# atoms-ufrj/atomsmm

Measured on AMD Instinct MI355X. Metric: ns/day on 100k-atom TIP3P RESPA box; near-nonbonded HBM GB/s vs 8 TB/s peak, higher is better.
Workload: dtype f64

## Files before the change

### atomsmm_amd/csrc/abi.hip

```cpp
#include <algorithm>
#include <cmath>
#include <cstring>
#include <numeric>

#include "amm_ctx.h"
#include "cluster.h"

int amm_pair_setup_grid(amm_ctx *ctx, PairForce *pf);
static bool amm_family_allows_cluster(int family, int flags) {
    const bool tab_family = family == AMM_NEAR_NONE || family == AMM_NEAR_SHIFT || family == AMM_NEAR_FSWITCH || family == AMM_DAMPED || family == AMM_NONBONDED;
    return tab_family && !(flags & (AMM_GROUP_LJ | AMM_GROUP_Q));
}
int amm_bonded_arity(int kind);
int amm_bonded_npar(int kind);

static thread_local std::string g_error;
void amm_set_error(const std::string &msg) { g_error = msg; }

static PairForce *get_pair(amm_ctx *ctx, int id) {
    if (!ctx || id < 0 || id >= (int)ctx->forces.size() || ctx->forces[id].type != 1) {
        amm_set_error("invalid pair force id");
        return nullptr;
    }
    return ctx->forces[id].pair;
// ... 1758 lines not shown
        amm_set_error("amm_set_option: null argument");
        return 1;
    }
    const std::string k(name);
    const int v = (int)value;
    if (k == "cluster") ctx->opt_cluster = v;
    else if (k == "hybrid") ctx->opt_hybrid = v;
    else if (k == "small_group") ctx->opt_small_group = v;
    else if (k == "mixed_terms") ctx->opt_mixed_terms = v;
    else if (k == "rest_skin_factor") ctx->opt_rest_skin_factor = value;
    else if (k == "tab") ctx->opt_tab = v;
    else if (k == "site_trips") ctx->site_trips = v != 0;
    else if (k == "lanes_per_row") ctx->opt_lpa = v;
    else if (k == "build_parts") ctx->opt_parts = v;
    else if (k == "build_split") ctx->opt_build_split = v;
    else if (k == "unroll") ctx->opt_unroll = v;
    else if (k == "dual_unroll") ctx->opt_dual_unroll = v;
    else if (k == "tab_block") ctx->opt_tab_bs = v;
    else if (k == "tab_dual_block") ctx->opt_tab_dual_bs = v;
    else if (k == "no_dual") ctx->opt_no_dual = v;
    else if (k == "fuse_rows") ctx->opt_fuse_rows = v;
    else if (k == "row_phases") ctx->opt_row_phases = v;
    else if (k == "group_candidates") ctx->opt_group_candidates = v;
    else if (k == "positions_private") ctx->opt_positions_private = v;
    else if (k == "site_tab") ctx->opt_site_tab = v;
    else if (k == "no_defer") ctx->opt_no_defer = v;
    else if (k == "terms_from") ctx->opt_terms_from = v;
    else if (k == "no_term_lanes") ctx->opt_no_term_lanes = v;
    else if (k == "fuse_epilogue") ctx->opt_fuse_epilogue = v;
    else if (k == "comm_timeout") ctx->opt_comm_timeout = value;
// ... 63 lines not shown
```

### atomsmm_amd/csrc/amm_ctx.h

```cpp
#pragma once
#include <hip/hip_runtime.h>

#include <cstdint>
#include <string>
#include <vector>

#include "../../include/atomsmm_hip.h"

#define AMM_WAVE 64
#define AMM_MAX_PRE 6
#define AMM_DERIV_LAMBDA 1024
#define AMM_MAX_GROUPS 33

void amm_set_error(const std::string &msg);
#define AMM_HIP(call)                                                                            \
    do {                                                                                         \
        hipError_t e_ = (call);                                                                  \
        if (e_ != hipSuccess) {                                                                  \
            amm_set_error(std::string(#call) + ": " + hipGetErrorString(e_));                    \
            return 1;                                                                            \
        }                                                                                        \
    } while (0)

struct PairTab {
// ... 253 lines not shown
    int opt_chargeless = 1;
    int opt_fuse_epilogue = 1;
    const EpiPlan *epi_request = nullptr;
    bool epi_done = false;
    long long n_epilogues = 0;
    long long n_state_exchanges = 0;
    std::vector<const double *> own_only;
    long long n_copies_current = 0;
    int opt_cluster = 1;
    int opt_hybrid = 1;
    double opt_rest_skin_factor = 2.0;
    int opt_mixed_terms = 1;
    int opt_small_group = 1;
    bool creating_rest = false;
    int opt_tab = 1;
    int opt_build_split = 0;
    int opt_lpa = 0, opt_parts = 0, opt_unroll = 2, opt_dual_unroll = 2, opt_tab_bs = 0, opt_tab_dual_bs = 0;
    int opt_site_tab = 1;
    CZeroRows zero_rows = CZeroRows{0, nullptr, nullptr, nullptr};
    int opt_positions_private = 0;
    int opt_group_candidates = 1;
    int opt_row_phases = 1;
    int opt_fuse_rows = 1;
    int opt_no_dual = 0, opt_no_defer = 0, opt_terms_from = 8192, opt_no_term_lanes = 0;
    ListWatch watched[AMM_MAX_WATCH];
    int n_watched = 0;
    int device = 0;
    hipStream_t stream = nullptr;
    Box box;
    int rank = 0, world = 1;
// ... 111 lines not shown
```

### atomsmm_amd/csrc/cluster.h

```cpp
#pragma once
#include "amm_ctx.h"

struct ClusterList {
    int nc = 0;
    const int *d_first = nullptr;
    const int *d_rest = nullptr;
    int nrest = 0;
    bool built = false;
    CellGrid grid;
    int capc = 0;
    int parts = 1;
    int *d_slice_cells = nullptr;
    int split_parts = 0;
    double rext = 0;
    double rlist_build = 0, rnear_build = 0, skin = 0;
    int *d_cell_count = nullptr, *d_cell_start = nullptr, *d_cell_members = nullptr;
    int *d_cperm = nullptr;
    int *d_aperm = nullptr;
    float4 *d_pos4f = nullptr;
    double *d_xref = nullptr;
    int c_begin = 0, c_end = 0;
    int cap = 0;
    int lpa = 8;
    int *d_nl = nullptr, *d_nnb = nullptr, *d_nnb_near = nullptr;
    int *d_flags = nullptr;
    unsigned long long *d_counters = nullptr;
    unsigned long long *d_blockstats = nullptr;
    int *d_ticket = nullptr;
    long checked_epoch = -1, pre_epoch = -1;
    const double *checked_pos = nullptr, *pre_pos = nullptr;
    PairForce *sorted_for = nullptr;
// ... 19 lines not shown
```

### atomsmm_amd/csrc/cluster.hip

```cpp
#include <algorithm>
#include <cmath>
#include <cstdio>
#include <cstdlib>
#include <cstring>
#include <type_traits>
#include <vector>

#include "amm_ctx.h"
#include "bonded_terms.h"
#include "cluster.h"
#include "device_utils.h"
#include "pair_math.h"
#include "pair_tab.h"

#ifndef AMM_EXP_NOLJ
#define AMM_EXP_NOLJ 0
#endif

__device__ double amm_erfcx_table_dev_c[AMM_ERFCX_NI * AMM_ERFCX_NC];
static bool g_erfcx_uploaded_c[64] = {false};

void amm_cluster_classify(int n, const std::vector<int> &ptr, const std::vector<int> &idx, std::vector<int> &mol_first, std::vector<int> &rest) {
    mol_first.clear();
    rest.clear();
// ... 77 lines not shown
#pragma unroll
    for (int k = 0; k < 3; ++k) sh[k] = cwrap1(pos[3 * i0 + k], box.L[k], box.invL[k]) - pos[3 * i0 + k];
#pragma unroll
    for (int a = 0; a < 3; ++a) {
        const int i = i0 + a;
        double4 p;
        p.x = csorted_image(pos[3 * i], pos[3 * i0], sh[0], box.L[0], box.invL[0]);
        p.y = csorted_image(pos[3 * i + 1], pos[3 * i0 + 1], sh[1], box.L[1], box.invL[1]);
        p.z = csorted_image(pos[3 * i + 2], pos[3 * i0 + 2], sh[2], box.L[2], box.invL[2]);
        p.w = q[i];
        posq_s[3 * c + a] = p;
        lj_s[3 * c + a] = make_double2(hsig[i], seps2[i]);
    }
}

__global__ void __launch_bounds__(256) k_csort_gather(int ncell, int nc, const int *__restrict__ start, const int *__restrict__ members,
                                                      int capc, int *cperm, int *aperm, const double *__restrict__ pos, Box box,
                                                      float4 *pos4f, const int *flags, int *wflags, int force, const double *__restrict__ q,
                                                      const double *__restrict__ hsig, const double *__restrict__ seps2, double4 *posq_s,
                                                      double2 *lj_s, float rext, const double *__restrict__ site_eps,
                                                      const int *__restrict__ first, CZeroRows Z, int copies_current, double *xref,
                                                      int c_begin, int c_end, int *slice_cells) {
    const int gid = blockIdx.x * blockDim.x + threadIdx.x;
    if (gid < Z.n) {
        const int i = Z.idx[gid];
        if (Z.f0) Z.f0[3 * i] = Z.f0[3 * i + 1] = Z.f0[3 * i + 2] = 0.0;
        if (Z.f1) Z.f1[3 * i] = Z.f1[3 * i + 1] = Z.f1[3 * i + 2] = 0.0;
    }
    if (!force && !flags[0]) {
        if (!copies_current && posq_s && gid < nc) cgather_one(gid, cfirst(first, cperm[gid]), pos, box, q, hsig, seps2, posq_s, lj_s);
        return;
    }
    const int wave = gid >> 6, lane = threadIdx.x & 63;
    if (wave >= ncell) return;
    const int b = start[wave];
    const int cnt = min(start[wave + 1] - b, capc);
    if (lane == 0 && c_begin < c_end) {
        if (b <= c_begin && c_begin < start[wave + 1]) slice_cells[0] = wave;
        if (b <= c_end - 1 && c_end - 1 < start[wave + 1]) slice_cells[1] = wave;
    }
    const int *mem = members + (size_t)wave * capc;
    for (int a0 = 0; a0 < cnt; a0 += 64) {
        const int a = a0 + lane;
        const int me = a < cnt ? mem[a] : 0x7fffffff;
        int rank = 0;
        for (int k0 = 0; k0 < cnt; k0 += 64) {
            const int kk = k0 + lane;
            const int other = kk < cnt ? mem[kk] : 0x7fffffff;
            const int nk = min(64, cnt - k0);
            for (int jj = 0; jj < nk; ++jj) rank += __builtin_amdgcn_readlane(other, jj) < me;
        }
        if (a >= cnt) continue;
        const int sl = b + rank;
        cperm[sl] = me;
        const int i0 = cfirst(first, me);
        double sh[3], p0[3];
#pragma unroll
        for (int k = 0; k < 3; ++k) {
            p0[k] = pos[3 * i0 + k];
            sh[k] = cwrap1(p0[k], box.L[k], box.invL[k]) - p0[k];
        }
        float ext2 = 0.f;
        int sites = 0;
        float4 pf[3];
#pragma unroll
        for (int t = 0; t < 3; ++t) {
            const int i = i0 + t;
            aperm[3 * sl + t] = i;
            const double x = csorted_image(pos[3 * i], p0[0], sh[0], box.L[0], box.invL[0]);
            const double y = csorted_image(pos[3 * i + 1], p0[1], sh[1], box.L[1], box.invL[1]);
// ... 7 lines not shown
            const float dx = pf[t].x - pf[0].x, dy = pf[t].y - pf[0].y, dz = pf[t].z - pf[0].z;
            ext2 = fmaxf(ext2, dx * dx + dy * dy + dz * dz);
            if (site_eps[i] != 0.0) sites |= 1 << t;
            if (posq_s) {
                posq_s[3 * sl + t] = make_double4(x, y, z, q[i]);
                lj_s[3 * sl + t] = make_double2(hsig[i], seps2[i]);
            }
        }
        const float ext = sqrtf(ext2) * 1.000001f + 1e-6f;
        if (!(ext <= rext)) wflags[7] = 1;
        pf[0].w = ext;
        pf[1].w = __int_as_float(sites);
        pos4f[3 * sl] = pf[0];
        pos4f[3 * sl + 1] = pf[1];
        pos4f[3 * sl + 2] = pf[2];
    }
}

struct CBoxF {
    float L[3], invL[3];
};

#ifndef CB_BATCH
#define CB_BATCH 5
#endif
#define CB_COARSE 256
#define CB_QCAP 256
__device__ __forceinline__ int cq_wrap(int i) { return i & (CB_QCAP - 1); }
typedef float v2f __attribute__((ext_vector_type(2)));

__device__ void cfinish_build_block(int *flags, unsigned long long *counters, const unsigned long long *blockstats, int nblocks, int count_only) {
    __shared__ unsigned long long sh_part[4][3];
    unsigned long long sum = 0, mx = 0, nr = 0;
    for (int b0 = threadIdx.x; b0 < nblocks; b0 += 8 * 256) {
        unsigned long long v[8][3];
#pragma unroll
        for (int j = 0; j < 8; ++j) {
            const int b = b0 + j * 256;
            const bool in = b < nblocks;
#pragma unroll
            for (int q = 0; q < 3; ++q) v[j][q] = in ? amm_ld_l2(&blockstats[3 * (in ? b : 0) + q]) : 0ull;
        }
#pragma unroll
// ... 15 lines not shown
    }
    __syncthreads();
    if (threadIdx.x == 0) {
        flags[2] = (int)max(max(sh_part[0][1], sh_part[1][1]), max(sh_part[2][1], sh_part[3][1]));
        counters[1] = sh_part[0][0] + sh_part[1][0] + sh_part[2][0] + sh_part[3][0];
        counters[2] = sh_part[0][2] + sh_part[1][2] + sh_part[2][2] + sh_part[3][2];
        if (!count_only) {
            flags[0] = 0;
            flags[AMM_FLAG_FAR] = 0;
            counters[0] += 1;
        }
    }
}

#ifndef CB_WAVES
#define CB_WAVES 5
#endif
#define CB_OCC __attribute__((amdgpu_waves_per_eu(CB_WAVES)))
#ifdef AMM_CBS_TIMING
__device__ unsigned long long g_cbs_t[8];
#define CBS_STAMP(i) do { const unsigned long long now_ = wall_clock64(); if (w == 0 && lane == 0) atomicAdd(&g_cbs_t[i], now_ - t_last); t_last = now_; } while (0)
#else
#define CBS_STAMP(i) do { } while (0)
#endif
template <bool COUNT_ONLY, bool RINT, bool SLICE = false>
__global__ void __launch_bounds__(256) __attribute__((amdgpu_waves_per_eu(SLICE ? 3 : CB_WAVES))) k_cbuild(int c_begin, int c_end, int parts, const int *__restrict__ cell_start,
                                                const float4 *__restrict__ pos4f, CBoxF box, CellGrid g, float rlist, float rnear2, int cap,
                                                int *nl, int *nnb, int *nnb_near, int *flags, unsigned long long *blockstats,
                                                unsigned long long *counters, int *ticket, int force, const int *slice_cells) {
    if (!force && !flags[0]) return;
    __shared__ int s_rstart[4][128];
    __shared__ int s_rpref[4][128];
    __shared__ float s_rshift[4][3][128];
    __shared__ int s_q[4][CB_BATCH][CB_QCAP];
    __shared__ unsigned char s_coarse[4][CB_COARSE];
    const int lane = threadIdx.x & 63, w = threadIdx.x >> 6;
    const int wave = __builtin_amdgcn_readfirstlane((int)((blockIdx.x * blockDim.x + threadIdx.x) >> 6));
    const float FAR = 1.0e9f;
    const float rlist2 = rlist * rlist;
    unsigned long long wsum = 0, wnear = 0;
    int wmax = 0;
    const int first_cell = SLICE ? __builtin_amdgcn_readfirstlane(slice_cells[0]) : 0;
    const int nunits = SLICE ? (__builtin_amdgcn_readfirstlane(slice_cells[1]) - first_cell + 1) * parts : g.ncell * parts;
    int unit = wave;
#ifdef AMM_CBS_TIMING
    unsigned long long t_last = wall_clock64(), t_drain = 0, n_drain = 0;
#endif
    do {
    const int c = unit < nunits ? first_cell + unit / parts : g.ncell, part = unit % parts;
    int a_begin = 0, a_end = 0;
    if (c < g.ncell) {
        const int cb0 = __builtin_amdgcn_readfirstlane(cell_start[c]), cb1 = __builtin_amdgcn_readfirstlane(cell_start[c + 1]);
        const int per = (cb1 - cb0 + parts - 1) / parts;
        a_begin = max(cb0 + part * per, c_begin);
        a_end = min(min(cb0 + (part + 1) * per, cb1), c_end);
    }
    if (a_begin < a_end) {
        const int ncx = g.nc[0], ncy = g.nc[1], ncz = g.nc[2];
        const int cx = c % ncx, cy = (c / ncx) % ncy, cz = c / (ncx * ncy);
        const int nsx = g.nstencil[0], nsy = g.nstencil[1], ne = nsx * nsy * g.nstencil[2];
        int total;
        {
            int ecs[2] = {0, 0}, len[2] = {0, 0}, inc[2];
            float esx[2] = {0.f, 0.f}, esy[2] = {0.f, 0.f}, esz[2] = {0.f, 0.f};
#pragma unroll
            for (int hh = 0; hh < 2; ++hh) {
                const int e = lane + 64 * hh;
                if (e < ne) {
                    const int ox = e % nsx, oy = (e / nsx) % nsy, oz = e / (nsx * nsy);
                    int nz = ncz < 2 * g.h[2] + 1 ? oz : cz - g.h[2] + oz;
                    esz[hh] = nz < 0 ? -box.L[2] : (nz >= ncz ? box.L[2] : 0.f);
                    nz = nz < 0 ? nz + ncz : (nz >= ncz ? nz - ncz : nz);
                    int ny = ncy < 2 * g.h[1] + 1 ? oy : cy - g.h[1] + oy;
                    esy[hh] = ny < 0 ? -box.L[1] : (ny >= ncy ? box.L[1] : 0.f);
                    ny = ny < 0 ? ny + ncy : (ny >= ncy ? ny - ncy : ny);
                    int nx = ncx < 2 * g.h[0] + 1 ? ox : cx - g.h[0] + ox;
                    esx[hh] = nx < 0 ? -box.L[0] : (nx >= ncx ? box.L[0] : 0.f);
                    nx = nx < 0 ? nx + ncx : (nx >= ncx ? nx - ncx : nx);
                    const int cc = (nz * ncy + ny) * ncx + nx;
                    ecs[hh] = cell_start[cc];
                    len[hh] = cell_start[cc + 1] - ecs[hh];
                }
                inc[hh] = len[hh];
                for (int off = 1; off < 64; off <<= 1) {
                    const int v = __shfl_up(inc[hh], off);
                    if (lane >= off) inc[hh] += v;
                }
            }
            const int lower = __builtin_amdgcn_readlane(inc[0], 63);
            total = lower + __builtin_amdgcn_readlane(inc[1], 63);
#pragma unroll
            for (int hh = 0; hh < 2; ++hh) {
                s_rstart[w][lane + 64 * hh] = ecs[hh];
                s_rpref[w][lane + 64 * hh] = (hh ? lower : 0) + inc[hh] - len[hh];
                s_rshift[w][0][lane + 64 * hh] = esx[hh];
                s_rshift[w][1][lane + 64 * hh] = esy[hh];
                s_rshift[w][2][lane + 64 * hh] = esz[hh];
            }
            __builtin_amdgcn_fence(__ATOMIC_RELEASE, "wavefront");
            __builtin_amdgcn_wave_barrier();
            __builtin_amdgcn_fence(__ATOMIC_ACQUIRE, "wavefront");
        }
        int cshift = 3;
        while (((total + 127) >> cshift) > CB_COARSE) ++cshift;
#pragma unroll
        for (int q = 0; q < CB_COARSE / 64; ++q) {
            const int idx = (lane + 64 * q) << cshift;
            int r = 0;
#pragma unroll
            for (int step = 64; step > 0; step >>= 1)
                if (s_rpref[w][r + step] <= idx) r += step;
            s_coarse[w][lane + 64 * q] = (unsigned char)r;
        }
        __builtin_amdgcn_fence(__ATOMIC_RELEASE, "wavefront");
        __builtin_amdgcn_wave_barrier();
        __builtin_amdgcn_fence(__ATOMIC_ACQUIRE, "wavefront");
#ifdef AMM_CBS_TIMING
        if (SLICE && lane == 0) { atomicAdd(&g_cbs_t[7], 1ull); atomicAdd(&g_cbs_t[0], wall_clock64() - t_last); }
#endif
        for (int tb = a_begin; tb < a_end; tb += CB_BATCH) {
            const int nt = min(CB_BATCH, a_end - tb);
            float4 my = make_float4(0.f, 0.f, 0.f, 0.f);
            if (lane < 3 * nt) my = pos4f[3 * tb + lane];
            int row_cnt = 0;
            int q_head = 0, q_cnt = 0;
            auto rl = [&](float v, int l) { return __int_as_float(__builtin_amdgcn_readlane(__float_as_int(v), l)); };
            auto drain = [&](int t, int n) {
#ifdef AMM_CBS_TIMING
                const unsigned long long t_d0 = wall_clock64();
                n_drain++;
#endif
                const int head = __builtin_amdgcn_readlane(q_head, t);
                int slot[2];
                bool v[2];
                float4 A[2][3];
#pragma unroll
                for (int u = 0; u < 2; ++u) {
                    const bool v0 = lane + 64 * u < n;
                    slot[u] = v0 ? s_q[w][t][cq_wrap(head + lane + 64 * u)] : tb + t;
                    v[u] = v0 && slot[u] != tb + t;
                }
// ... 66 lines not shown
                        row_cnt = lane == t ? c2 + nn_ + ((np_ - nn_) << 16) : row_cnt;
                    }
                }
                q_head = lane == t ? cq_wrap(head + n) : q_head;
                q_cnt = lane == t ? q_cnt - n : q_cnt;
#ifdef AMM_CBS_TIMING
                t_drain += wall_clock64() - t_d0;
#endif
            };
            auto fetch = [&](int cb, float4 (&cand)[2], int (&js)[2]) {
#pragma unroll
                for (int u = 0; u < 2; ++u) {
                    const int idx = cb + u * 64 + lane;
                    const bool in = idx < total;
                    int r = s_coarse[w][idx >> cshift];
                    while (r < 127 && s_rpref[w][r + 1] <= idx) ++r;
                    const int slot = in ? s_rstart[w][r] + idx - s_rpref[w][r] : 0;
                    float4 q = pos4f[3 * slot];
                    if (!RINT) {
                        const float sx = s_rshift[w][0][r], sy = s_rshift[w][1][r], sz = s_rshift[w][2][r];
                        q.x = in ? q.x + sx : FAR;
                        q.y = in ? q.y + sy : FAR;
                        q.z = in ? q.z + sz : FAR;
                    } else if (!in) {
                        q.w = -1.0e9f;
                    }
                    cand[u] = q;
                    js[u] = slot;
                }
            };
            float4 cand[2], cand_n[2];
            int js[2], js_n[2];
            fetch(0, cand, js);
            const float plim_l = my.w + rlist;
            for (int cb = 0; cb < total; cb += 128) {
// ... 1293 lines not shown
    }
    return 0;
}

static int cluster_chain(amm_ctx *ctx, PairForce *L, ClusterList *cl, const double *d_pos, int force, bool count_only, PairForce *gather_for,
                         CZeroRows Z = CZeroRows{0, nullptr, nullptr, nullptr}, int copies_current = 0, bool skip_assign = false) {
    hipStream_t st = ctx->stream;
    const int nc = cl->nc;
    if (!skip_assign)
        hipLaunchKernelGGL(k_cassign, dim3((nc + cl->nrest + 255) / 256), dim3(256), 0, st, nc, d_pos, ctx->box, cl->grid, cl->d_cell_count, cl->d_cell_start,
                           cl->d_cell_members, cl->capc, count_only ? (double *)nullptr : cl->d_xref, cl->d_flags, cl->d_ticket, force, cl->d_first,
                           cl->d_rest, cl->nrest);
    if (!cl->d_cell_members) return 0;
    PairForce *gf = gather_for;
    const long sort_threads = std::max(std::max((long)cl->grid.ncell * 64, gf ? (long)nc : 0L), (long)Z.n);
    hipLaunchKernelGGL(k_csort_gather, dim3((unsigned)((sort_threads + 255) / 256)), dim3(256), 0, st, cl->grid.ncell, nc, cl->d_cell_start,
                       cl->d_cell_members, cl->capc, cl->d_cperm, cl->d_aperm, d_pos, ctx->box, cl->d_pos4f, cl->d_flags, cl->d_flags, force,
                       gf ? gf->d_q : nullptr, gf ? gf->d_hsig : nullptr, gf ? gf->d_seps2 : nullptr, gf ? gf->d_posq_s : (double4 *)nullptr,
                       gf ? gf->d_lj_s : (double2 *)nullptr, (float)cl->rext, L->d_seps2, cl->d_first, Z, copies_current,
                       count_only ? (double *)nullptr : cl->d_xref, cl->c_begin, cl->c_end, cl->d_slice_cells);
    const bool slice = cl->c_end - cl->c_begin < cl->nc;
    const bool split = cl->split_parts > 0 && !count_only;
    const int ncell_grid = slice ? (int)std::min<long>(cl->grid.ncell, (5L * cl->grid.ncell) / (4L * std::max(1, ctx->world)) + 4) : cl->grid.ncell;
    const long threads = (long)ncell_grid * cl->parts * 64;
    dim3 grid(split ? (unsigned)(ncell_grid * cl->split_parts) : (unsigned)((threads + 255) / 256));
    CBoxF bf;
    for (int k = 0; k < 3; ++k) {
        bf.L[k] = (float)ctx->box.L[k];
        bf.invL[k] = (float)ctx->box.invL[k];
    }
    const float rl = (float)cl->rlist_build;
    const float rn2 = cl->rnear_build > 0 ? (float)(cl->rnear_build * cl->rnear_build) : 3.0e38f;
    const bool use_rint = cl->grid.nc[0] < 5 || cl->grid.nc[1] < 5 || cl->grid.nc[2] < 5;
#define AMM_LAUNCH_CBUILD(CO, RI)                                                                                                   \
    do {                                                                                                                            \
        if (slice)                                                                                                                  \
            hipLaunchKernelGGL((k_cbuild<CO, RI, true>), grid, dim3(256), 0, st, cl->c_begin, cl->c_end, cl->parts, cl->d_cell_start,    \
                               cl->d_pos4f, bf, cl->grid, rl, rn2, cl->cap, cl->d_nl, cl->d_nnb, cl->d_nnb_near, cl->d_flags,            \
                               cl->d_blockstats, cl->d_counters, cl->d_ticket + AMM_TICKET_INTS, force, cl->d_slice_cells);              \
        else                                                                                                                        \
            hipLaunchKernelGGL((k_cbuild<CO, RI, false>), grid, dim3(256), 0, st, cl->c_begin, cl->c_end, cl->parts, cl->d_cell_start,   \
                               cl->d_pos4f, bf, cl->grid, rl, rn2, cl->cap, cl->d_nl, cl->d_nnb, cl->d_nnb_near, cl->d_flags,            \
                               cl->d_blockstats, cl->d_counters, cl->d_ticket + AMM_TICKET_INTS, force, cl->d_slice_cells);              \
    } while (0)
#define AMM_LAUNCH_CBUILD_SPLIT(RI)                                                                                                  \
    hipLaunchKernelGGL((k_cbuild_split<RI>), grid, dim3(256), 0, st, cl->c_begin, cl->c_end, cl->split_parts, cl->d_cell_start,     \
                       cl->d_pos4f, bf, cl->grid, rl, rn2, cl->cap, cl->d_nl, cl->d_nnb, cl->d_nnb_near, cl->d_flags, cl->d_blockstats,  \
                       cl->d_counters, cl->d_ticket + AMM_TICKET_INTS, force, cl->d_slice_cells)
    if (count_only) {
        if (use_rint) AMM_LAUNCH_CBUILD(true, true);
        else AMM_LAUNCH_CBUILD(true, false);
    } else if (split) {
        if (use_rint) AMM_LAUNCH_CBUILD_SPLIT(true);
        else AMM_LAUNCH_CBUILD_SPLIT(false);
    } else {
        if (use_rint) AMM_LAUNCH_CBUILD(false, true);
        else AMM_LAUNCH_CBUILD(false, false);
    }
// ... 37 lines not shown
    const double ext = cluster_extent_host(ctx, d_pos, n, nc, L->h_mol_first);
    if (!(ext >= 0.0) || !(ext == ext)) {
        amm_set_error("molecule-row list: cannot read the positions (or NaN positions)");
        return 1;
    }
    cl->rext = std::max(1.5 * ext, ext + 0.05);
    if (cluster_setup_grid(ctx, cl, L->desc.rc)) return 1;
    const int per = (nc + ctx->world - 1) / ctx->world;
    cl->c_begin = std::min(nc, ctx->rank * per);
    cl->c_end = std::min(nc, cl->c_begin + per);
    const size_t ns = (size_t)std::max(cl->c_end - cl->c_begin, 1);
    const int ncell = cl->grid.ncell;
    AMM_HIP(hipMalloc(&cl->d_cell_count, sizeof(int) * (ncell + 1)));
    AMM_HIP(hipMemset(cl->d_cell_count, 0, sizeof(int) * (ncell + 1)));
    AMM_HIP(hipMalloc(&cl->d_cell_start, sizeof(int) * (ncell + 1)));
    AMM_HIP(hipMalloc(&cl->d_cperm, sizeof(int) * nc));
    AMM_HIP(hipMalloc(&cl->d_aperm, sizeof(int) * 3 * (size_t)nc));
    AMM_HIP(hipMalloc(&cl->d_pos4f, sizeof(float4) * 3 * (size_t)nc));
    AMM_HIP(hipMalloc(&cl->d_xref, sizeof(double) * 3 * (size_t)n));
    AMM_HIP(hipMalloc(&cl->d_nnb, sizeof(int) * ns));
    AMM_HIP(hipMalloc(&cl->d_nnb_near, sizeof(int) * ns));
    AMM_HIP(hipMalloc(&cl->d_flags, sizeof(int) * 16));
    AMM_HIP(hipMemset(cl->d_flags, 0, sizeof(int) * 16));
    AMM_HIP(hipMalloc(&cl->d_ticket, sizeof(int) * 4 * AMM_TICKET_INTS));
    AMM_HIP(hipMemset(cl->d_ticket, 0, sizeof(int) * 4 * AMM_TICKET_INTS));
    AMM_HIP(hipMalloc(&cl->d_counters, sizeof(unsigned long long) * 8));
    AMM_HIP(hipMemset(cl->d_counters, 0, sizeof(unsigned long long) * 8));
    AMM_HIP(hipMalloc(&cl->d_slice_cells, sizeof(int) * 2));
    AMM_HIP(hipMemset(cl->d_slice_cells, 0, sizeof(int) * 2));
    int lpa = 4;
// ... 81 lines not shown
    if (copies_current) ctx->n_copies_current++;
    if (cl->checked_epoch == ctx->pos_epoch && cl->checked_pos == d_pos && !L->force_rebuild_c) {
    } else {
        if (!(cl->pre_epoch == ctx->pos_epoch && cl->pre_pos == d_pos))
            hipLaunchKernelGGL(k_ccheck_displacement, dim3((n + 255) / 256), dim3(256), 0, st, n, d_pos, cl->d_xref, 0.25 * cl->skin * cl->skin,
                               cl->d_flags);
        const int forced = L->force_rebuild_c ? 1 : 0;
        L->force_rebuild_c = false;
        const bool assigned = !forced && cl->assigned_epoch == ctx->pos_epoch && cl->assigned_pos == d_pos;
        if (cluster_chain(ctx, L, cl, d_pos, forced, false, pf, Z, copies_current, assigned)) return 1;
        gathered = true;
    }
    cl->checked_epoch = ctx->pos_epoch;
    cl->checked_pos = d_pos;
    if (!gathered && !copies_current)
        hipLaunchKernelGGL(k_csort_gather, dim3((std::max(cl->nc, Z.n) + 255) / 256), dim3(256), 0, st, cl->grid.ncell, cl->nc, cl->d_cell_start,
                           cl->d_cell_members, cl->capc, cl->d_cperm, cl->d_aperm, d_pos, ctx->box, cl->d_pos4f, cl->d_flags + 8, cl->d_flags, 0,
                           pf->d_q, pf->d_hsig, pf->d_seps2, pf->d_posq_s, pf->d_lj_s, (float)cl->rext, L->d_seps2, cl->d_first, Z, 0, (double *)nullptr, 0, 0, (int *)nullptr);
    cl->sorted_for = pf;
    cl->sorted_epoch = ctx->pos_epoch;
    cl->sorted_pos = d_pos;
    const int nrows = cl->c_end - cl->c_begin;
    const int per_c = (cl->nc + ctx->world - 1) / ctx->world, per = 3 * per_c, nf = guest ? 2 : 1;
    double *out = d_force, *gout = g_force;
    auto ss_bytes_of = [](const PairForce *p) { return (p->d_tab_ss && p->pc.tab.ss_first >= 0) ? (p->pc.tab.nint - p->pc.tab.ss_first) * AMM_TAB_STRIDE : 0; };
    auto plan_fits = [&]() {
        if (!(plan && plan->kind == 0 && ctx->opt_fuse_epilogue && !accumulate && !cl->d_first && cl->nrest == 0 && plan->bs && plan->bs->mol3_ok &&
              plan->bs->finalized && plan->bs->ncomp == cl->nc && plan->f0 && plan->npre <= AMM_MAX_PRE && ctx->d_x == d_pos && ctx->d_v &&
              plan->f0 != d_force && plan->f0 != g_force)) return false;
        if (guest && !(!g_accumulate && g_force != d_force && ctx->opt_fuse_rows && pf == L && cl->rnear_build > 0)) return false;
        return true;
    };
    bool state_mode = false;
// ... 293 lines not shown
                    const double dx = amm_min_image(pi.x - pj.x, A.box.L[0], A.box.invL[0]);
                    const double dy = amm_min_image(pi.y - pj.y, A.box.L[1], A.box.invL[1]);
                    const double dz = amm_min_image(pi.z - pj.z, A.box.L[2], A.box.invL[2]);
                    cnt += (dx * dx + dy * dy + dz * dz < r2w) ? 1ull : 0ull;
                }
        }
    }
    for (int off = 32; off > 0; off >>= 1) cnt += __shfl_xor(cnt, off);
    if ((threadIdx.x & 63) == 0 && cnt) atomicAdd(out, cnt);
}

int amm_cluster_count_within_impl(amm_ctx *ctx, PairForce *pf, const double *d_pos, double r_within, long long *count) {
    PairForce *L = pf->host ? pf->host : pf;
    ClusterList *cl = L->cl;
    hipStream_t st = ctx->stream;
    hipLaunchKernelGGL(k_csort_gather, dim3((cl->nc + 255) / 256), dim3(256), 0, st, cl->grid.ncell, cl->nc, cl->d_cell_start, cl->d_cell_members,
                       cl->capc, cl->d_cperm, cl->d_aperm, d_pos, ctx->box, cl->d_pos4f, cl->d_flags + 8, cl->d_flags, 0, pf->d_q, pf->d_hsig,
                       pf->d_seps2, pf->d_posq_s, pf->d_lj_s, (float)cl->rext, L->d_seps2, cl->d_first, CZeroRows{0, nullptr, nullptr, nullptr}, 0, (double *)nullptr, 0, 0, (int *)nullptr);
    if (cl->sorted_for == pf) {
        cl->sorted_epoch = ctx->pos_epoch;
        cl->sorted_pos = d_pos;
    }
    CPairArgs A;
    std::memset(&A, 0, sizeof(A));
    A.c_begin = cl->c_begin;
    A.nrows = cl->c_end - cl->c_begin;
    A.cap = cl->cap;
    A.nl = cl->d_nl;
    A.nnb = (pf == L) ? cl->d_nnb : cl->d_nnb_near;
    A.nnb_total = nullptr;
    if (pf == L && cl->rnear_build > 0) {
        A.nnb = cl->d_nnb_near;
        A.nnb_total = cl->d_nnb;
// ... 58 lines not shown
#ifdef AMM_CBS_TIMING
    {
        unsigned long long t[8];
        const bool got = hipMemcpyFromSymbol(t, HIP_SYMBOL(g_cbs_t), sizeof(t)) == hipSuccess && t[7];
        if (got && cl->split_parts == 0)
            fprintf(stderr, "k_cbuild<SLICE>: %llu busy wavefronts, mean: prologue %.2f us, whole %.2f us, in drains %.2f us (%.2f drains)\n", t[7], t[0] / 100.0 / t[7],
                    t[1] / 100.0 / t[7], t[2] / 100.0 / t[7], (double)t[3] / t[7]);
        if (got && cl->split_parts > 0)
            fprintf(stderr, "k_cbuild_split, first wavefront of %llu busy blocks, mean clocks (100 MHz): prologue %.2f | pass 1 %.2f wait %.2f | pass 2 %.2f wait %.2f | copy %.2f wait %.2f us\n",
                    t[7], t[0] / 100.0 / t[7], t[1] / 100.0 / t[7], t[2] / 100.0 / t[7], t[3] / 100.0 / t[7], t[4] / 100.0 / t[7], t[5] / 100.0 / t[7], t[6] / 100.0 / t[7]);
    }
#endif
    for (void *q : {(void *)cl->d_spec_count[0], (void *)cl->d_spec_count[1], (void *)cl->d_spec_ticket})
        if (q) (void)hipFree(q);
    if (cl->d_slice_cells) (void)hipFree(cl->d_slice_cells);
    void *ptrs[] = {cl->d_cell_count, cl->d_cell_start, cl->d_cell_members, cl->d_cperm, cl->d_aperm, cl->d_pos4f, cl->d_xref, cl->d_nl,
                    cl->d_nnb, cl->d_nnb_near, cl->d_flags, cl->d_counters, cl->d_blockstats, cl->d_ticket};
    for (void *p : ptrs)
        if (p) (void)hipFree(p);
    delete cl;
    return 0;
}
```

Baseline: 1081.

## Cull neighbor-cell octants per cluster batch during neighbor list build

The sort/gather kernel now orders clusters within each cell by octant (sub-cell half in x, y, z) and records octant boundaries plus the maximum cluster extent per cell. The list build kernel then computes, for each batch of row clusters, a bounding box and drops stencil-cell octants whose gap exceeds the list cutoff, building candidate runs only from kept pieces. This aims to cut the number of candidate distance checks in the build, at the cost of extra sort-key work, a per-batch (rather than per-row-cell) run setup, and slightly lower occupancy (CB_WAVES from 5 to 4).

```diff
diff --git a/atomsmm_amd/csrc/abi.hip b/atomsmm_amd/csrc/abi.hip
--- a/atomsmm_amd/csrc/abi.hip
+++ b/atomsmm_amd/csrc/abi.hip
@@ -1796,6 +1796,7 @@
     else if (k == "lanes_per_row") ctx->opt_lpa = v;
     else if (k == "build_parts") ctx->opt_parts = v;
     else if (k == "build_split") ctx->opt_build_split = v;
+    else if (k == "build_cull") ctx->opt_build_cull = v;
     else if (k == "unroll") ctx->opt_unroll = v;
     else if (k == "dual_unroll") ctx->opt_dual_unroll = v;
     else if (k == "tab_block") ctx->opt_tab_bs = v;
diff --git a/atomsmm_amd/csrc/amm_ctx.h b/atomsmm_amd/csrc/amm_ctx.h
--- a/atomsmm_amd/csrc/amm_ctx.h
+++ b/atomsmm_amd/csrc/amm_ctx.h
@@ -291,6 +291,7 @@
     int opt_small_group = 1;
     bool creating_rest = false;
     int opt_tab = 1;
+    int opt_build_cull = 1;
     int opt_build_split = 0;
     int opt_lpa = 0, opt_parts = 0, opt_unroll = 2, opt_dual_unroll = 2, opt_tab_bs = 0, opt_tab_dual_bs = 0;
     int opt_site_tab = 1;
diff --git a/atomsmm_amd/csrc/cluster.h b/atomsmm_amd/csrc/cluster.h
--- a/atomsmm_amd/csrc/cluster.h
+++ b/atomsmm_amd/csrc/cluster.h
@@ -15,6 +15,7 @@
     double rext = 0;
     double rlist_build = 0, rnear_build = 0, skin = 0;
     int *d_cell_count = nullptr, *d_cell_start = nullptr, *d_cell_members = nullptr;
+    int *d_cell_oct = nullptr;
     int *d_cperm = nullptr;
     int *d_aperm = nullptr;
     float4 *d_pos4f = nullptr;
diff --git a/atomsmm_amd/csrc/cluster.hip b/atomsmm_amd/csrc/cluster.hip
--- a/atomsmm_amd/csrc/cluster.hip
+++ b/atomsmm_amd/csrc/cluster.hip
@@ -115,13 +115,26 @@
     }
 }
 
-__global__ void __launch_bounds__(256) k_csort_gather(int ncell, int nc, const int *__restrict__ start, const int *__restrict__ members,
+__device__ __forceinline__ unsigned csort_key(int m, const int *__restrict__ first, const double *__restrict__ pos, const Box &box,
+                                              const CellGrid &g, const int (&cc)[3]) {
+    const int i0 = cfirst(first, m);
+    unsigned o = 0;
+#pragma unroll
+    for (int k = 0; k < 3; ++k) {
+        const double w = cwrap1(pos[3 * i0 + k], box.L[k], box.invL[k]);
+        const int h = (w == w) ? (int)(w * (2.0 * g.inv_cw[k])) - 2 * cc[k] : 0;
+        o |= (h >= 1 ? 1u : 0u) << k;
+    }
+    return (o << 29) | (unsigned)m;
+}
+
+__global__ void __launch_bounds__(256) k_csort_gather(CellGrid g, int nc, const int *__restrict__ start, const int *__restrict__ members,
                                                       int capc, int *cperm, int *aperm, const double *__restrict__ pos, Box box,
                                                       float4 *pos4f, const int *flags, int *wflags, int force, const double *__restrict__ q,
                                                       const double *__restrict__ hsig, const double *__restrict__ seps2, double4 *posq_s,
                                                       double2 *lj_s, float rext, const double *__restrict__ site_eps,
                                                       const int *__restrict__ first, CZeroRows Z, int copies_current, double *xref,
-                                                      int c_begin, int c_end, int *slice_cells) {
+                                                      int c_begin, int c_end, int *slice_cells, int *cell_oct) {
     const int gid = blockIdx.x * blockDim.x + threadIdx.x;
     if (gid < Z.n) {
         const int i = Z.idx[gid];
@@ -133,28 +146,37 @@
         return;
     }
     const int wave = gid >> 6, lane = threadIdx.x & 63;
-    if (wave >= ncell) return;
+    if (wave >= g.ncell) return;
     const int b = start[wave];
     const int cnt = min(start[wave + 1] - b, capc);
+    const int cc[3] = {wave % g.nc[0], (wave / g.nc[0]) % g.nc[1], wave / (g.nc[0] * g.nc[1])};
     if (lane == 0 && c_begin < c_end) {
         if (b <= c_begin && c_begin < start[wave + 1]) slice_cells[0] = wave;
         if (b <= c_end - 1 && c_end - 1 < start[wave + 1]) slice_cells[1] = wave;
     }
     const int *mem = members + (size_t)wave * capc;
+    int below = 0;
+    float ext_max = 0.f;
     for (int a0 = 0; a0 < cnt; a0 += 64) {
         const int a = a0 + lane;
-        const int me = a < cnt ? mem[a] : 0x7fffffff;
+        const unsigned me = a < cnt ? csort_key(mem[a], first, pos, box, g, cc) : 0xffffffffu;
         int rank = 0;
         for (int k0 = 0; k0 < cnt; k0 += 64) {
             const int kk = k0 + lane;
-            const int other = kk < cnt ? mem[kk] : 0x7fffffff;
+            const unsigned other = k0 == a0 ? me : (kk < cnt ? csort_key(mem[kk], first, pos, box, g, cc) : 0xffffffffu);
             const int nk = min(64, cnt - k0);
-            for (int jj = 0; jj < nk; ++jj) rank += __builtin_amdgcn_readlane(other, jj) < me;
+            for (int jj = 0; jj < nk; ++jj) rank += (unsigned)__builtin_amdgcn_readlane((int)other, jj) < me;
+        }
+#pragma unroll
+        for (int k = 1; k < 8; ++k) {
+            const int nbelow = __popcll(__builtin_amdgcn_ballot_w64(a < cnt && (me >> 29) < (unsigned)k));
+            below += lane == k ? nbelow : 0;
         }
         if (a >= cnt) continue;
         const int sl = b + rank;
-        cperm[sl] = me;
-        const int i0 = cfirst(first, me);
+        const int me_m = (int)(me & 0x1fffffffu);
+        cperm[sl] = me_m;
+        const int i0 = cfirst(first, me_m);
         double sh[3], p0[3];
 #pragma unroll
         for (int k = 0; k < 3; ++k) {
@@ -192,7 +214,13 @@
         pos4f[3 * sl] = pf[0];
         pos4f[3 * sl + 1] = pf[1];
         pos4f[3 * sl + 2] = pf[2];
-    }
+        ext_max = fmaxf(ext_max, ext);
+    }
+    if (!cell_oct) return;
+    for (int off = 32; off > 0; off >>= 1) ext_max = fmaxf(ext_max, __shfl_xor(ext_max, off));
+    if (cnt < start[wave + 1] - b) ext_max = 1.0e18f;
+    if (lane == 0) cell_oct[8 * wave] = __float_as_int(ext_max);
+    if (lane >= 1 && lane < 8) cell_oct[8 * wave + lane] = b + below;
 }
 
 struct CBoxF {
@@ -203,8 +231,36 @@
 #define CB_BATCH 5
 #endif
 #define CB_COARSE 256
+#define CB_RUNS 256
 #define CB_QCAP 256
 __device__ __forceinline__ int cq_wrap(int i) { return i & (CB_QCAP - 1); }
+__device__ __forceinline__ int cpieces(const int (&r)[9], int m) {
+    int np = 0;
+    bool open = false;
+#pragma unroll
+    for (int o = 0; o < 8; ++o) {
+        const int l = r[o + 1] - r[o];
+        const bool kept = (m >> o) & 1;
+        np += (l > 0 && kept && !open) ? 1 : 0;
+        open = l > 0 ? kept : open;
+    }
+    return np;
+}
+__device__ __forceinline__ int ckept(const int (&r)[9], int m) {
+    int len = 0;
+#pragma unroll
+    for (int o = 0; o < 8; ++o) len += ((m >> o) & 1) ? r[o + 1] - r[o] : 0;
+    return len;
+}
+__device__ __forceinline__ void cscan2(int &a, int &b, int lane) {
+    for (int off = 1; off < 64; off <<= 1) {
+        const int v = __shfl_up(a, off), u = __shfl_up(b, off);
+        if (lane >= off) {
+            a += v;
+            b += u;
+        }
+    }
+}
 typedef float v2f __attribute__((ext_vector_type(2)));
 
 __device__ void cfinish_build_block(int *flags, unsigned long long *counters, const unsigned long long *blockstats, int nblocks, int count_only) {
@@ -250,7 +306,7 @@
 }
 
 #ifndef CB_WAVES
-#define CB_WAVES 5
+#define CB_WAVES 4
 #endif
 #define CB_OCC __attribute__((amdgpu_waves_per_eu(CB_WAVES)))
 #ifdef AMM_CBS_TIMING
@@ -263,11 +319,12 @@
 __global__ void __launch_bounds__(256) __attribute__((amdgpu_waves_per_eu(SLICE ? 3 : CB_WAVES))) k_cbuild(int c_begin, int c_end, int parts, const int *__restrict__ cell_start,
                                                 const float4 *__restrict__ pos4f, CBoxF box, CellGrid g, float rlist, float rnear2, int cap,
                                                 int *nl, int *nnb, int *nnb_near, int *flags, unsigned long long *blockstats,
-                                                unsigned long long *counters, int *ticket, int force, const int *slice_cells) {
+                                                unsigned long long *counters, int *ticket, int force, const int *slice_cells,
+                                                const int *__restrict__ cell_oct, int cull) {
     if (!force && !flags[0]) return;
-    __shared__ int s_rstart[4][128];
-    __shared__ int s_rpref[4][128];
-    __shared__ float s_rshift[4][3][128];
+    __shared__ int s_rpref[4][CB_RUNS];
+    __shared__ int s_rdelta[4][CB_RUNS];
+    __shared__ unsigned char s_rcode[4][CB_RUNS];
     __shared__ int s_q[4][CB_BATCH][CB_QCAP];
     __shared__ unsigned char s_coarse[4][CB_COARSE];
     const int lane = threadIdx.x & 63, w = threadIdx.x >> 6;
@@ -295,65 +352,6 @@
         const int ncx = g.nc[0], ncy = g.nc[1], ncz = g.nc[2];
         const int cx = c % ncx, cy = (c / ncx) % ncy, cz = c / (ncx * ncy);
         const int nsx = g.nstencil[0], nsy = g.nstencil[1], ne = nsx * nsy * g.nstencil[2];
-        int total;
-        {
-            int ecs[2] = {0, 0}, len[2] = {0, 0}, inc[2];
-            float esx[2] = {0.f, 0.f}, esy[2] = {0.f, 0.f}, esz[2] = {0.f, 0.f};
-#pragma unroll
-            for (int hh = 0; hh < 2; ++hh) {
-                const int e = lane + 64 * hh;
-                if (e < ne) {
-                    const int ox = e % nsx, oy = (e / nsx) % nsy, oz = e / (nsx * nsy);
-                    int nz = ncz < 2 * g.h[2] + 1 ? oz : cz - g.h[2] + oz;
-                    esz[hh] = nz < 0 ? -box.L[2] : (nz >= ncz ? box.L[2] : 0.f);
-                    nz = nz < 0 ? nz + ncz : (nz >= ncz ? nz - ncz : nz);
-                    int ny = ncy < 2 * g.h[1] + 1 ? oy : cy - g.h[1] + oy;
-                    esy[hh] = ny < 0 ? -box.L[1] : (ny >= ncy ? box.L[1] : 0.f);
-                    ny = ny < 0 ? ny + ncy : (ny >= ncy ? ny - ncy : ny);
-                    int nx = ncx < 2 * g.h[0] + 1 ? ox : cx - g.h[0] + ox;
-                    esx[hh] = nx < 0 ? -box.L[0] : (nx >= ncx ? box.L[0] : 0.f);
-                    nx = nx < 0 ? nx + ncx : (nx >= ncx ? nx - ncx : nx);
-                    const int cc = (nz * ncy + ny) * ncx + nx;
-                    ecs[hh] = cell_start[cc];
-                    len[hh] = cell_start[cc + 1] - ecs[hh];
-                }
-                inc[hh] = len[hh];
-                for (int off = 1; off < 64; off <<= 1) {
-                    const int v = __shfl_up(inc[hh], off);
-                    if (lane >= off) inc[hh] += v;
-                }
-            }
-            const int lower = __builtin_amdgcn_readlane(inc[0], 63);
-            total = lower + __builtin_amdgcn_readlane(inc[1], 63);
-#pragma unroll
-            for (int hh = 0; hh < 2; ++hh) {
-                s_rstart[w][lane + 64 * hh] = ecs[hh];
-                s_rpref[w][lane + 64 * hh] = (hh ? lower : 0) + inc[hh] - len[hh];
-                s_rshift[w][0][lane + 64 * hh] = esx[hh];
-                s_rshift[w][1][lane + 64 * hh] = esy[hh];
-                s_rshift[w][2][lane + 64 * hh] = esz[hh];
-            }
-            __builtin_amdgcn_fence(__ATOMIC_RELEASE, "wavefront");
-            __builtin_amdgcn_wave_barrier();
-            __builtin_amdgcn_fence(__ATOMIC_ACQUIRE, "wavefront");
-        }
-        int cshift = 3;
-        while (((total + 127) >> cshift) > CB_COARSE) ++cshift;
-#pragma unroll
-        for (int q = 0; q < CB_COARSE / 64; ++q) {
-            const int idx = (lane + 64 * q) << cshift;
-            int r = 0;
-#pragma unroll
-            for (int step = 64; step > 0; step >>= 1)
-                if (s_rpref[w][r + step] <= idx) r += step;
-            s_coarse[w][lane + 64 * q] = (unsigned char)r;
-        }
-        __builtin_amdgcn_fence(__ATOMIC_RELEASE, "wavefront");
-        __builtin_amdgcn_wave_barrier();
-        __builtin_amdgcn_fence(__ATOMIC_ACQUIRE, "wavefront");
-#ifdef AMM_CBS_TIMING
-        if (SLICE && lane == 0) { atomicAdd(&g_cbs_t[7], 1ull); atomicAdd(&g_cbs_t[0], wall_clock64() - t_last); }
-#endif
         for (int tb = a_begin; tb < a_end; tb += CB_BATCH) {
             const int nt = min(CB_BATCH, a_end - tb);
             float4 my = make_float4(0.f, 0.f, 0.f, 0.f);
@@ -361,6 +359,151 @@
             int row_cnt = 0;
             int q_head = 0, q_cnt = 0;
             auto rl = [&](float v, int l) { return __int_as_float(__builtin_amdgcn_readlane(__float_as_int(v), l)); };
+            int total, cshift;
+            {
+                float bc[3], bh[3], exti = 0.f, cwf[3];
+#pragma unroll
+                for (int k = 0; k < 3; ++k) {
+                    cwf[k] = (float)g.cw[k];
+                    asm volatile("" : "+v"(cwf[k]));
+                }
+                {
+                    float lo[3] = {FAR, FAR, FAR}, hi[3] = {-FAR, -FAR, -FAR};
+                    for (int t = 0; t < nt; ++t) {
+                        const float p[3] = {rl(my.x, 3 * t), rl(my.y, 3 * t), rl(my.z, 3 * t)};
+#pragma unroll
+                        for (int k = 0; k < 3; ++k) {
+                            lo[k] = fminf(lo[k], p[k]);
+                            hi[k] = fmaxf(hi[k], p[k]);
+                        }
+                        exti = fmaxf(exti, rl(my.w, 3 * t));
+                    }
+#pragma unroll
+                    for (int k = 0; k < 3; ++k) {
+                        bc[k] = 0.5f * (lo[k] + hi[k]);
+                        bh[k] = 0.5f * (hi[k] - lo[k]) + 0.25f * cwf[k] + 1.0e-5f * box.L[k];
+                    }
+                }
+                int rb[2][9], keep[2], code[2];
+                int lane_b = lane;
+                asm volatile("" : "+v"(lane_b));
+#pragma unroll
+                for (int hh = 0; hh < 2; ++hh) {
+                    const int e = 2 * lane_b + hh;
+                    keep[hh] = 0;
+                    code[hh] = 0;
+#pragma unroll
+                    for (int o = 0; o < 9; ++o) rb[hh][o] = 0;
+                    if (e < ne) {
+                        const int os[3] = {e % nsx, (e / nsx) % nsy, e / (nsx * nsy)}, cs[3] = {cx, cy, cz};
+                        int n3[3];
+                        float sh[3];
+#pragma unroll
+                        for (int k = 0; k < 3; ++k) {
+                            int nk = g.nc[k] < 2 * g.h[k] + 1 ? os[k] : cs[k] - g.h[k] + os[k];
+                            const int cd = nk < 0 ? 1 : (nk >= g.nc[k] ? 2 : 0);
+                            code[hh] |= cd << (2 * k);
+                            sh[k] = RINT ? 0.f : (cd == 1 ? -box.L[k] : (cd == 2 ? box.L[k] : 0.f));
+                            n3[k] = nk < 0 ? nk + g.nc[k] : (nk >= g.nc[k] ? nk - g.nc[k] : nk);
+                        }
+                        const int cc = (n3[2] * ncy + n3[1]) * ncx + n3[0];
+                        const int4 ra = *(const int4 *)(cell_oct + 8 * (size_t)cc), rc = *(const int4 *)(cell_oct + 8 * (size_t)cc + 4);
+                        rb[hh][0] = cell_start[cc];
+                        rb[hh][1] = ra.y;
+                        rb[hh][2] = ra.z;
+                        rb[hh][3] = ra.w;
+                        rb[hh][4] = rc.x;
+                        rb[hh][5] = rc.y;
+                        rb[hh][6] = rc.z;
+                        rb[hh][7] = rc.w;
+                        rb[hh][8] = cell_start[cc + 1];
+                        keep[hh] = 0xff;
+                        if (cull) {
+                            const float lim = (rlist + exti + __int_as_float(ra.x)) * 1.00001f;
+                            float g2[3][2];
+#pragma unroll
+                            for (int k = 0; k < 3; ++k)
+#pragma unroll
+                                for (int hf = 0; hf < 2; ++hf) {
+                                    float d = ((float)(2 * n3[k] + hf) + 0.5f) * (0.5f * cwf[k]) + sh[k] - bc[k];
+                                    if (RINT) d -= box.L[k] * rintf(d * box.invL[k]);
+                                    const float gap = fmaxf(fabsf(d) - bh[k], 0.f);
+                                    g2[k][hf] = gap * gap;
+                                }
+                            keep[hh] = 0;
+#pragma unroll
+                            for (int o = 0; o < 8; ++o)
+                                keep[hh] |= (g2[0][o & 1] + g2[1][(o >> 1) & 1] + g2[2][o >> 2] < lim * lim) ? 1 << o : 0;
+                        }
+                    }
+                }
+                int np = cpieces(rb[0], keep[0]) + cpieces(rb[1], keep[1]);
+                int len = ckept(rb[0], keep[0]) + ckept(rb[1], keep[1]);
+                int inp = np, ilen = len;
+                cscan2(inp, ilen, lane);
+                int npieces = __builtin_amdgcn_readlane(inp, 63);
+                if (npieces > CB_RUNS - 2) {
+#pragma unroll
+                    for (int hh = 0; hh < 2; ++hh)
+                        if (keep[hh]) keep[hh] = ((2 << (31 - __builtin_clz(keep[hh]))) - 1) & ~((1 << __builtin_ctz(keep[hh])) - 1);
+                    np = cpieces(rb[0], keep[0]) + cpieces(rb[1], keep[1]);
+                    len = ckept(rb[0], keep[0]) + ckept(rb[1], keep[1]);
+                    inp = np;
+                    ilen = len;
+                    cscan2(inp, ilen, lane);
+                    npieces = __builtin_amdgcn_readlane(inp, 63);
+                }
+                total = __builtin_amdgcn_readlane(ilen, 63);
+                int idx = inp - np, pref = ilen - len;
+#pragma unroll
+                for (int hh = 0; hh < 2; ++hh) {
+                    int s0 = 0;
+                    bool open = false;
+#pragma unroll
+                    for (int o = 0; o <= 8; ++o) {
+                        const int l = o < 8 ? rb[hh][o + 1] - rb[hh][o] : 1;
+                        const bool kept = o < 8 && ((keep[hh] >> o) & 1);
+                        if (l > 0 && open && !kept) {
+                            s_rpref[w][idx] = pref;
+                            s_rdelta[w][idx] = s0 - pref;
+                            s_rcode[w][idx] = (unsigned char)code[hh];
+                            pref += rb[hh][o] - s0;
+                            ++idx;
+                        }
+                        if (l > 0 && kept && !open) s0 = rb[hh][o];
+                        open = l > 0 ? kept : open;
+                    }
+                }
+#pragma unroll
+                for (int q = 0; q < CB_RUNS / 64; ++q) {
+                    const int k = lane + 64 * q;
+                    if (k >= npieces) {
+                        s_rpref[w][k] = k == npieces ? total : 0x7fffffff;
+                        s_rdelta[w][k] = 0;
+                        s_rcode[w][k] = 0;
+                    }
+                }
+                __builtin_amdgcn_fence(__ATOMIC_RELEASE, "wavefront");
+                __builtin_amdgcn_wave_barrier();
+                __builtin_amdgcn_fence(__ATOMIC_ACQUIRE, "wavefront");
+                cshift = 3;
+                while (((total + 127) >> cshift) >= CB_COARSE) ++cshift;
+#pragma unroll
+                for (int q = 0; q < CB_COARSE / 64; ++q) {
+                    const int at = (lane + 64 * q) << cshift;
+                    int r = 0;
+#pragma unroll
+                    for (int step = CB_RUNS / 2; step > 0; step >>= 1)
+                        if (s_rpref[w][r + step] <= at) r += step;
+                    s_coarse[w][lane + 64 * q] = (unsigned char)r;
+                }
+                __builtin_amdgcn_fence(__ATOMIC_RELEASE, "wavefront");
+                __builtin_amdgcn_wave_barrier();
+                __builtin_amdgcn_fence(__ATOMIC_ACQUIRE, "wavefront");
+            }
+#ifdef AMM_CBS_TIMING
+            if (SLICE && lane == 0 && tb == a_begin) { atomicAdd(&g_cbs_t[7], 1ull); atomicAdd(&g_cbs_t[0], wall_clock64() - t_last); }
+#endif
             auto drain = [&](int t, int n) {
 #ifdef AMM_CBS_TIMING
                 const unsigned long long t_d0 = wall_clock64();
@@ -457,11 +600,14 @@
                     const int idx = cb + u * 64 + lane;
                     const bool in = idx < total;
                     int r = s_coarse[w][idx >> cshift];
-                    while (r < 127 && s_rpref[w][r + 1] <= idx) ++r;
-                    const int slot = in ? s_rstart[w][r] + idx - s_rpref[w][r] : 0;
+                    while (r < CB_RUNS - 2 && s_rpref[w][r + 1] <= idx) ++r;
+                    const int slot = in ? idx + s_rdelta[w][r] : 0;
                     float4 q = pos4f[3 * slot];
                     if (!RINT) {
-                        const float sx = s_rshift[w][0][r], sy = s_rshift[w][1][r], sz = s_rshift[w][2][r];
+                        const int cd = s_rcode[w][r];
+                        const float sx = (cd & 1) ? -box.L[0] : ((cd & 2) ? box.L[0] : 0.f);
+                        const float sy = (cd & 4) ? -box.L[1] : ((cd & 8) ? box.L[1] : 0.f);
+                        const float sz = (cd & 16) ? -box.L[2] : ((cd & 32) ? box.L[2] : 0.f);
                         q.x = in ? q.x + sx : FAR;
                         q.y = in ? q.y + sy : FAR;
                         q.z = in ? q.z + sz : FAR;
@@ -1785,11 +1931,12 @@
     if (!cl->d_cell_members) return 0;
     PairForce *gf = gather_for;
     const long sort_threads = std::max(std::max((long)cl->grid.ncell * 64, gf ? (long)nc : 0L), (long)Z.n);
-    hipLaunchKernelGGL(k_csort_gather, dim3((unsigned)((sort_threads + 255) / 256)), dim3(256), 0, st, cl->grid.ncell, nc, cl->d_cell_start,
+    hipLaunchKernelGGL(k_csort_gather, dim3((unsigned)((sort_threads + 255) / 256)), dim3(256), 0, st, cl->grid, nc, cl->d_cell_start,
                        cl->d_cell_members, cl->capc, cl->d_cperm, cl->d_aperm, d_pos, ctx->box, cl->d_pos4f, cl->d_flags, cl->d_flags, force,
                        gf ? gf->d_q : nullptr, gf ? gf->d_hsig : nullptr, gf ? gf->d_seps2 : nullptr, gf ? gf->d_posq_s : (double4 *)nullptr,
                        gf ? gf->d_lj_s : (double2 *)nullptr, (float)cl->rext, L->d_seps2, cl->d_first, Z, copies_current,
-                       count_only ? (double *)nullptr : cl->d_xref, cl->c_begin, cl->c_end, cl->d_slice_cells);
+                       count_only ? (double *)nullptr : cl->d_xref, cl->c_begin, cl->c_end, cl->d_slice_cells, cl->d_cell_oct);
+    const int cull = ctx->opt_build_cull ? 1 : 0;
     const bool slice = cl->c_end - cl->c_begin < cl->nc;
     const bool split = cl->split_parts > 0 && !count_only;
     const int ncell_grid = slice ? (int)std::min<long>(cl->grid.ncell, (5L * cl->grid.ncell) / (4L * std::max(1, ctx->world)) + 4) : cl->grid.ncell;
@@ -1808,11 +1955,13 @@
         if (slice)                                                                                                                  \
             hipLaunchKernelGGL((k_cbuild<CO, RI, true>), grid, dim3(256), 0, st, cl->c_begin, cl->c_end, cl->parts, cl->d_cell_start,    \
                                cl->d_pos4f, bf, cl->grid, rl, rn2, cl->cap, cl->d_nl, cl->d_nnb, cl->d_nnb_near, cl->d_flags,            \
-                               cl->d_blockstats, cl->d_counters, cl->d_ticket + AMM_TICKET_INTS, force, cl->d_slice_cells);              \
+                               cl->d_blockstats, cl->d_counters, cl->d_ticket + AMM_TICKET_INTS, force, cl->d_slice_cells,               \
+                               cl->d_cell_oct, cull);                                                                                   \
         else                                                                                                                        \
             hipLaunchKernelGGL((k_cbuild<CO, RI, false>), grid, dim3(256), 0, st, cl->c_begin, cl->c_end, cl->parts, cl->d_cell_start,   \
                                cl->d_pos4f, bf, cl->grid, rl, rn2, cl->cap, cl->d_nl, cl->d_nnb, cl->d_nnb_near, cl->d_flags,            \
-                               cl->d_blockstats, cl->d_counters, cl->d_ticket + AMM_TICKET_INTS, force, cl->d_slice_cells);              \
+                               cl->d_blockstats, cl->d_counters, cl->d_ticket + AMM_TICKET_INTS, force, cl->d_slice_cells,               \
+                               cl->d_cell_oct, cull);                                                                                   \
     } while (0)
 #define AMM_LAUNCH_CBUILD_SPLIT(RI)                                                                                                  \
     hipLaunchKernelGGL((k_cbuild_split<RI>), grid, dim3(256), 0, st, cl->c_begin, cl->c_end, cl->split_parts, cl->d_cell_start,     \
@@ -1880,6 +2029,8 @@
     AMM_HIP(hipMalloc(&cl->d_cell_count, sizeof(int) * (ncell + 1)));
     AMM_HIP(hipMemset(cl->d_cell_count, 0, sizeof(int) * (ncell + 1)));
     AMM_HIP(hipMalloc(&cl->d_cell_start, sizeof(int) * (ncell + 1)));
+    AMM_HIP(hipMalloc(&cl->d_cell_oct, sizeof(int) * 8 * (size_t)ncell));
+    AMM_HIP(hipMemset(cl->d_cell_oct, 0, sizeof(int) * 8 * (size_t)ncell));
     AMM_HIP(hipMalloc(&cl->d_cperm, sizeof(int) * nc));
     AMM_HIP(hipMalloc(&cl->d_aperm, sizeof(int) * 3 * (size_t)nc));
     AMM_HIP(hipMalloc(&cl->d_pos4f, sizeof(float4) * 3 * (size_t)nc));
@@ -1991,9 +2142,10 @@
     cl->checked_epoch = ctx->pos_epoch;
     cl->checked_pos = d_pos;
     if (!gathered && !copies_current)
-        hipLaunchKernelGGL(k_csort_gather, dim3((std::max(cl->nc, Z.n) + 255) / 256), dim3(256), 0, st, cl->grid.ncell, cl->nc, cl->d_cell_start,
+        hipLaunchKernelGGL(k_csort_gather, dim3((std::max(cl->nc, Z.n) + 255) / 256), dim3(256), 0, st, cl->grid, cl->nc, cl->d_cell_start,
                            cl->d_cell_members, cl->capc, cl->d_cperm, cl->d_aperm, d_pos, ctx->box, cl->d_pos4f, cl->d_flags + 8, cl->d_flags, 0,
-                           pf->d_q, pf->d_hsig, pf->d_seps2, pf->d_posq_s, pf->d_lj_s, (float)cl->rext, L->d_seps2, cl->d_first, Z, 0, (double *)nullptr, 0, 0, (int *)nullptr);
+                           pf->d_q, pf->d_hsig, pf->d_seps2, pf->d_posq_s, pf->d_lj_s, (float)cl->rext, L->d_seps2, cl->d_first, Z, 0, (double *)nullptr, 0, 0, (int *)nullptr,
+                           (int *)nullptr);
     cl->sorted_for = pf;
     cl->sorted_epoch = ctx->pos_epoch;
     cl->sorted_pos = d_pos;
@@ -2317,9 +2469,10 @@
     PairForce *L = pf->host ? pf->host : pf;
     ClusterList *cl = L->cl;
     hipStream_t st = ctx->stream;
-    hipLaunchKernelGGL(k_csort_gather, dim3((cl->nc + 255) / 256), dim3(256), 0, st, cl->grid.ncell, cl->nc, cl->d_cell_start, cl->d_cell_members,
+    hipLaunchKernelGGL(k_csort_gather, dim3((cl->nc + 255) / 256), dim3(256), 0, st, cl->grid, cl->nc, cl->d_cell_start, cl->d_cell_members,
                        cl->capc, cl->d_cperm, cl->d_aperm, d_pos, ctx->box, cl->d_pos4f, cl->d_flags + 8, cl->d_flags, 0, pf->d_q, pf->d_hsig,
-                       pf->d_seps2, pf->d_posq_s, pf->d_lj_s, (float)cl->rext, L->d_seps2, cl->d_first, CZeroRows{0, nullptr, nullptr, nullptr}, 0, (double *)nullptr, 0, 0, (int *)nullptr);
+                       pf->d_seps2, pf->d_posq_s, pf->d_lj_s, (float)cl->rext, L->d_seps2, cl->d_first, CZeroRows{0, nullptr, nullptr, nullptr}, 0, (double *)nullptr, 0, 0, (int *)nullptr,
+                       (int *)nullptr);
     if (cl->sorted_for == pf) {
         cl->sorted_epoch = ctx->pos_epoch;
         cl->sorted_pos = d_pos;
@@ -2408,7 +2561,7 @@
     for (void *q : {(void *)cl->d_spec_count[0], (void *)cl->d_spec_count[1], (void *)cl->d_spec_ticket})
         if (q) (void)hipFree(q);
     if (cl->d_slice_cells) (void)hipFree(cl->d_slice_cells);
-    void *ptrs[] = {cl->d_cell_count, cl->d_cell_start, cl->d_cell_members, cl->d_cperm, cl->d_aperm, cl->d_pos4f, cl->d_xref, cl->d_nl,
+    void *ptrs[] = {cl->d_cell_count, cl->d_cell_start, cl->d_cell_oct, cl->d_cell_members, cl->d_cperm, cl->d_aperm, cl->d_pos4f, cl->d_xref, cl->d_nl,
                     cl->d_nnb, cl->d_nnb_near, cl->d_flags, cl->d_counters, cl->d_blockstats, cl->d_ticket};
     for (void *p : ptrs)
         if (p) (void)hipFree(p);
```

Result: slower. 1067, median of 2 (-1.3%).
